# navallo/collision_avoidance

Hardware: AMD Instinct MI355X
Metric: agent-steps/sec (whole node), 4096 arenas x 64 agents per GPU (higher is better)
Workload: dtype f32

## Files before the change

collision_avoidance_amd/_lib.py:

```python
import ctypes as C
import os

from . import build as _build

OBS_DIM = 64
MAX_NEIGHBORS, MAX_OBST_NEIGHBORS, MAX_AGENTS = 16, 64, 1024
MAX_AGENTS_LARGE = 16384
CREATE_TILED = 1
CREATE_TILED_GRID = 4
CREATE_TILED_PARAMS = 16
CREATE_TILED_WIDE = 32
EDGE_GRID_MAX_EDGES, EDGE_GRID_MAX_ENTRIES = 65535, 1 << 22
DONE_XLESS, DONE_GOAL, DONE_REGOAL = 0, 1, 2
F_OBS, F_STATS, F_AUTORESET, F_NODONE, F_FREEZE = 1, 2, 4, 8, 16
F_CONTACT = 32
TRACE_POS, TRACE_VEL = 1, 2
SCN_CROWD, SCN_CIRCLE, SCN_DOORWAY, SCN_CONGESTED, SCN_INCOMING, SCN_BLOCKS, SCN_DEADLOCK, SCN_CROWD_SEPARATED = range(8)

(FLD_POS_X, FLD_POS_Y, FLD_VEL_X, FLD_VEL_Y, FLD_PREF_X, FLD_PREF_Y, FLD_GOAL_X, FLD_GOAL_Y,
 FLD_GOAL2_X, FLD_GOAL2_Y, FLD_REWARD, FLD_AGENT_DONE, FLD_ARRIVE_STEP, FLD_NB_COUNT, FLD_NB_IDX,
 FLD_OBST_COUNT, FLD_OBST_IDX, FLD_OBS, FLD_STEP_COUNT, FLD_ARENA_DONE, FLD_EPISODE,
 FLD_REGOAL_COUNT, FLD_ALAN_WEIGHTS, FLD_ALAN_TIMES, FLD_ALAN_ACTION, FLD_ARENA_STATS) = range(26)

EXPORTS = ("ca_create", "ca_destroy", "ca_last_error", "ca_set_stream", "ca_set_obstacles", "ca_init_scenario", "ca_set",
           "ca_get", "ca_field_ptr", "ca_bind_obs", "ca_reset", "ca_step", "ca_step_host", "ca_orca_step", "ca_observe", "ca_rollout",
           "ca_get_stats", "ca_reset_stats", "ca_sync", "ca_debug_math", "ca_profile", "ca_profile_read", "ca_launch_info",
           "ca_alan_configure", "ca_alan_step", "ca_alan_rollout", "ca_reset_masked", "ca_get_obstacles",
           "ca_set_obstacles_per_arena", "ca_get_obstacles_arena", "ca_solver_info", "ca_source_sha", "ca_host_alloc", "ca_host_free",
           "ca_step_packed", "ca_allow_obstacle_overflow", "ca_alan_configure_per_arena", "ca_alan_actions_arena",
           "ca_set_agent_params", "ca_get_agent_params", "ca_agent_params_info",
           "ca_set_agent_counts", "ca_get_agent_counts", "ca_agent_counts_info", "ca_create_ex", "ca_tiled_info", "ca_tiled_grid_info",
           "ca_rollout_trace", "ca_alan_rollout_trace", "ca_tiled_edge_grid", "ca_tiled_edge_grid_info", "ca_edge_grid_build",
           "ca_contacts", "ca_get_contacts", "ca_contacts_ptr",
           "ca_set_agent_sensing", "ca_get_agent_sensing", "ca_agent_sensing_info", "ca_nbr_seed_info",
           "ca_arena_gather", "ca_snapshot_create", "ca_snapshot_save", "ca_snapshot_load", "ca_snapshot_destroy",
           "ca_fork_bytes_per_arena", "ca_rollout_actions",
           "ca_policy_configure", "ca_policy_clear", "ca_policy_info", "ca_policy_actions", "ca_rollout_policy",
           "ca_nav_configure", "ca_nav_clear", "ca_nav_info", "ca_nav_get_field", "ca_nav_pref", "ca_rollout_nav", "ca_nav_mask_build")
POLICY_OUT_IDENTITY, POLICY_OUT_CLIP = 0, 1
POLICY_MAX_LAYERS, POLICY_MAX_WIDTH = 4, 128
NAV_MAX_CELLS, NAV_MAX_GOALS, NAV_MAX_LOOKAHEAD = 32768, 16, 8
NAV_STAY, NAV_NONE = 8, 9
NAV_OFFSETS = ((1, 0), (0, 1), (-1, 0), (0, -1), (1, 1), (-1, 1), (-1, -1), (1, -1))


class Config(C.Structure):
    _fields_ = [
        ("n_arenas", C.c_int32), ("n_agents", C.c_int32), ("arena_offset", C.c_int64),
        ("seed", C.c_uint64), ("reward_scale", C.c_double), ("time_step", C.c_float),
        ("neighbor_dist", C.c_float), ("max_neighbors", C.c_int32), ("time_horizon", C.c_float),
        ("time_horizon_obst", C.c_float), ("radius", C.c_float), ("max_speed", C.c_float),
        ("max_obst_neighbors", C.c_int32), ("max_step", C.c_int32), ("done_mode", C.c_int32),
        ("done_x_thresh", C.c_float), ("spawn_x0", C.c_float), ("spawn_x1", C.c_float),
        ("spawn_y0", C.c_float), ("spawn_y1", C.c_float), ("goal_x0", C.c_float),
        ("goal_x1", C.c_float), ("goal_y0", C.c_float), ("goal_y1", C.c_float),
    ]

# ... 111 lines not shown
    L.ca_nav_get_field.argtypes = [vp, i32, i32, vp, vp, vp, i32]
    L.ca_nav_pref.argtypes = [vp, vp, u32]
    L.ca_rollout_nav.argtypes = [vp, i32, u32, C.POINTER(Trace)]
    L.ca_nav_mask_build.argtypes = [vp, i32, C.c_float, C.c_float, C.c_float, i32, i32, C.c_float, vp, i32]
    L.ca_get_stats.argtypes = [vp, C.POINTER(Stats)]
    L.ca_reset_stats.argtypes = [vp]
    L.ca_sync.argtypes = [vp]
    L.ca_allow_obstacle_overflow.argtypes = [vp, i32]
    L.ca_debug_math.argtypes = [vp, i32, vp, vp, i32]
    L.ca_profile.argtypes = [vp, i32]
    L.ca_profile_read.argtypes = [vp, C.POINTER(i32), C.POINTER(C.c_float)]
    L.ca_launch_info.argtypes = [vp] + [C.POINTER(i32)] * 4
    L.ca_solver_info.argtypes = [vp, C.POINTER(i32), C.POINTER(i32)]
    L.ca_set_agent_params.argtypes = [vp, vp, vp, vp, vp, sz, i32]
    L.ca_get_agent_params.argtypes = [vp, vp, vp, vp, vp, sz, i32]
    L.ca_agent_params_info.argtypes = [vp, C.POINTER(i32)]
    L.ca_set_agent_counts.argtypes = [vp, vp, sz, i32]
    L.ca_get_agent_counts.argtypes = [vp, vp, sz, i32]
    L.ca_agent_counts_info.argtypes = [vp, C.POINTER(i32)]
    L.ca_set_agent_sensing.argtypes = [vp, vp, vp, sz, i32]
    L.ca_get_agent_sensing.argtypes = [vp, vp, vp, sz, i32]
    L.ca_agent_sensing_info.argtypes = [vp, C.POINTER(i32)]
    L.ca_nbr_seed_info.argtypes = [vp, C.POINTER(i32)]
    L.ca_arena_gather.argtypes = [vp, vp, sz, i32, u32]
    L.ca_snapshot_create.argtypes = [vp, C.POINTER(vp)]
    L.ca_snapshot_save.argtypes = [vp, vp]
    L.ca_snapshot_load.argtypes = [vp, vp, vp, sz, i32, u32]
    L.ca_snapshot_destroy.argtypes = [vp, vp]
    L.ca_fork_bytes_per_arena.argtypes = [vp, C.POINTER(sz)]
    L.ca_source_sha.argtypes = []
    L.ca_source_sha.restype = C.c_char_p
    for name in EXPORTS:
        if name not in ("ca_last_error", "ca_source_sha"):
            getattr(L, name).restype = C.c_int
    _lib = L
    return L


def edge_grid_build(edges_pq, rng):
    import numpy as np
    L = load()
    pq = np.ascontiguousarray(edges_pq, np.float32).reshape(-1, 4)
    d = EdgeGridDesc()
    ptr = pq.ctypes.data_as(C.c_void_p) if len(pq) else None
    check(L, None, L.ca_edge_grid_build(ptr, len(pq), float(rng), C.byref(d), None, 0, None, 0), "ca_edge_grid_build")
    cs, en = np.zeros(d.gx * d.gy + 1, np.uint32), np.zeros(max(1, d.n_entries), np.uint32)
# ... 20 lines not shown
```

collision_avoidance_amd/csrc/ca_common.h:

```cpp
#pragma once
#include "ca_math.h"
#include <type_traits>
#include <utility>

struct AlanArenaSets;
struct WideObstLists;
struct AgentParams;
struct ArenaCounts;
struct AgentSensing;
struct Trace;
struct ActionSeq;
struct SeededScan;

namespace ca {

template <class T, class... P> constexpr bool has_tag = (std::is_same_v<T, P> || ...);

constexpr int SMAX = 16;
constexpr int SWIDE = 64;
constexpr float EPS = 0.00001f;

struct ObstDev {
    float px, py, ux, uy;
    float qx, qy, qux, quy;
    float pux, puy;
    int next, prev;
    int convex, qconvex, pad0, pad1;
};
static_assert(sizeof(ObstDev) == 64, "edge record is one 64-byte line");

struct Line {
    V2 point, dir;
};

struct TraceDev;
// ... 259 lines not shown
```

collision_avoidance_amd/csrc/ca_env.hip:

```cpp
#include "../../include/ca_env.h"

#include <hip/hip_runtime.h>
#include <hip/hip_ext.h>

#include <algorithm>
#include <cmath>
#include <cstdarg>
#include <cstdlib>
#include <cstdio>
#include <cstring>
#include <string>
#include <vector>

#include "ca_kernels.h"
#include "ca_edge_grid_host.h"
#include "ca_nav_host.h"

using namespace ca;

struct StateSet {
    unsigned char* base = nullptr;
    unsigned char* alan = nullptr;
    int alan_nA = 0;
};
// ... 63 lines not shown
        int L = 0, P = 0, out_mode = 0, maxw = 0;
        int width[CA_POLICY_MAX_LAYERS + 1] = {0, 0, 0, 0, 0};
        float limit = 0.0f;
        unsigned wp_off[CA_POLICY_MAX_LAYERS] = {0, 0, 0, 0}, bp_off[CA_POLICY_MAX_LAYERS] = {0, 0, 0, 0}, wset = 0, bset = 0;
        float *d_wp = nullptr, *d_bp = nullptr, *act = nullptr;
        int* d_set = nullptr;
    } pol;
    struct Nav {
        bool on = false;
        float x0 = 0.0f, y0 = 0.0f, cell = 0.0f, ics = 0.0f, clearance = 0.0f;
        int gx = 0, gy = 0, G = 0, sets = 0, per_arena = 0, lookahead = 0, sweeps_max = 0, block = 0;
        float* d_dist = nullptr;
        unsigned char* d_next = nullptr;
        int* d_class = nullptr;
        std::vector<unsigned char> h_blocked;
    } nav;
    unsigned long long* ovf_host = nullptr;
    bool allow_overflow = false;
    int* d_order = nullptr;
    int P = 1, logP = 0, BS = 64, grid = 1, K = 0, S = 1;
    bool obs_dense_on = false;
    bool lists_trusted = true;
    int LS = 1, apb = 1, linv = 65536, dense = 0;
    struct { int reg_lines = -1, pair = -1, alan_fused = -1, nbr_seed = -1, nav_block = 0; } sw;
    int ST = 0, KT = 16;
    int SMX = 4;
    int max_edges = 0;
    int n_cus = 256;
    bool pair = false;
    size_t lds_p = 0;
    bool quad = false;
    bool quad_roll = false;
    int BSq = 64, grid_q = 1, SQ = 4;
    size_t lds_q = 0;
    size_t lds = 0;
    bool ap = false, quad_cfg = false, quad_roll_cfg = false;
    float* d_ap[4] = {nullptr, nullptr, nullptr, nullptr};
    float* d_ap_oct = nullptr;
    std::vector<float> h_ap[4];
    bool ac = false, ap_user = false;
    int* d_counts = nullptr;
    std::vector<int> h_counts;
    bool sens = false;
    float* d_as_nd = nullptr;
    unsigned char* d_as_k = nullptr;
    std::vector<float> h_as_nd;
    std::vector<int> h_as_k;
// ... 168 lines not shown
    c.trace = e->d_trace;
    c.actseq = e->d_actseq;
    c.as_neighbor_dist = e->sens ? e->d_as_nd : nullptr; c.as_max_neighbors = e->sens ? e->d_as_k : nullptr;
}

static void fill_args(ca_env* e, StepArgs& a, const float* actions, uint32_t flags) {
    const ca_config& c = e->cfg;
    a.pos_x = e->pos_x; a.pos_y = e->pos_y; a.vel_x = e->vel_x; a.vel_y = e->vel_y;
    a.pref_x = e->pref_x; a.pref_y = e->pref_y; a.goal_x = e->goal_x; a.goal_y = e->goal_y;
    a.counts = e->counts; a.nb_idx = e->nb_idx; a.obst_idx = e->obst_idx;
    a.arena_done = e->arena_done; a.arena_stats = e->arena_stats; a.cold = e->d_cold;
    a.obst = e->d_obst; a.tab_off = e->d_tab_off; a.actions = actions; a.alan = nullptr; a.alan_u = nullptr;
#ifdef CA_STAMPS
    a.order = e->d_order;
#endif
    a.reset_px = nullptr; a.reset_py = nullptr; a.reset_mask = nullptr; a.dbg = e->dbg;
    a.n_obst = e->h_tab_off.empty() ? (int)e->h_obst.size() : 0; a.A = c.n_arenas; a.N = c.n_agents; a.P = e->P; a.logP = e->logP;
    a.K = e->K; a.S = e->S; a.flags = flags; a.a0 = 0; a.a1 = c.n_arenas; a.T = 1;
    a.LS = e->LS; a.apb = e->apb; a.linv = e->linv; a.dense = e->dense; a.nb_hint = e->lists_trusted ? 1 : 0;
    a.time_step = c.time_step; a.neighbor_dist = c.neighbor_dist; a.time_horizon = c.time_horizon;
    a.time_horizon_obst = c.time_horizon_obst; a.radius = c.radius; a.max_speed = c.max_speed;
}

struct SolveLaunch { const void* fn; dim3 grid, block; size_t lds; bool seeded = false; };
template <class F> static const void* fn_ptr(F* f) { return reinterpret_cast<const void*>(f); }
template <int KMAX, int ST, int SMX, bool ALAN, class... PER>
static const void* step_fn_for(int BS, bool seed, bool* seeded) {
#if CA_NBR_SEED
    if (seed && BS == 64) { *seeded = true; return fn_ptr(&step_kernel<KMAX, 64, ST, SMX, ALAN, PER..., SeededScan>); }
#endif
    if constexpr (ALAN) {
        return BS == 64 ? fn_ptr(&step_kernel<KMAX, 64, ST, SMX, true, PER...>) : fn_ptr(&step_kernel<KMAX, 128, ST, SMX, true, PER...>);
    } else {
        switch (BS) {
            case 64: return fn_ptr(&step_kernel<KMAX, 64, ST, SMX>);
            case 128: return fn_ptr(&step_kernel<KMAX, 128, ST, SMX>);
            case 256: return fn_ptr(&step_kernel<KMAX, 256, ST, SMX>);
            case 512: return fn_ptr(&step_kernel<KMAX, 512, ST, SMX>);
            default: return fn_ptr(&step_kernel<KMAX, 1024, ST, SMX>);
        }
    }
}
template <int KMAX>
static const void* pair_fn_for(int BS) {
    return BS == 256 ? fn_ptr(&pair_kernel<KMAX, 256>) : fn_ptr(&pair_kernel<KMAX, 512>);
}
template <int KMAX, int SQ, bool ALAN, class... PER>
static const void* quad_fn_for(int BS) {
    switch (BS) {
        case 64: return fn_ptr(&quad_kernel<KMAX, 64, SQ, ALAN, PER...>);
        case 128: return fn_ptr(&quad_kernel<KMAX, 128, SQ, ALAN, PER...>);
        case 256: return fn_ptr(&quad_kernel<KMAX, 256, SQ, ALAN, PER...>);
// ... 22 lines not shown
    switch (BS) {
        case 64: return fn_ptr(&step_kernel<KMAX, 64, 0, SMAX, false, ArenaCounts>);
        case 128: return fn_ptr(&step_kernel<KMAX, 128, 0, SMAX, false, ArenaCounts>);
        case 256: return fn_ptr(&step_kernel<KMAX, 256, 0, SMAX, false, ArenaCounts>);
        case 512: return fn_ptr(&step_kernel<KMAX, 512, 0, SMAX, false, ArenaCounts>);
        default: return fn_ptr(&step_kernel<KMAX, 1024, 0, SMAX, false, ArenaCounts>);
    }
}
template <int KMAX, class... TAGS>
static const void* sens_fn_for(int BS) {
    switch (BS) {
        case 64: return fn_ptr(&step_kernel<KMAX, 64, 0, SMAX, false, TAGS...>);
        case 128: return fn_ptr(&step_kernel<KMAX, 128, 0, SMAX, false, TAGS...>);
        case 256: return fn_ptr(&step_kernel<KMAX, 256, 0, SMAX, false, TAGS...>);
        case 512: return fn_ptr(&step_kernel<KMAX, 512, 0, SMAX, false, TAGS...>);
        default: return fn_ptr(&step_kernel<KMAX, 1024, 0, SMAX, false, TAGS...>);
    }
}
template <class... TAGS>
static const void* sens_fn_of(const ca_env* e) {
    return e->KT == 5 ? sens_fn_for<5, TAGS...>(e->BS) : (e->KT == 16 ? sens_fn_for<16, TAGS...>(e->BS) : sens_fn_for<10, TAGS...>(e->BS));
}
template <bool ALAN, class... PER>
static const void* lane_fn_for(const ca_env* e, bool* seeded) {
    const bool sd = e->sw.nbr_seed != 0;
    if (e->sens) return e->ac ? sens_fn_of<ArenaCounts, AgentSensing>(e) : sens_fn_of<AgentSensing>(e);
    if (e->ac) return e->KT == 5 ? ac_fn_for<5>(e->BS, sd, seeded) : (e->KT == 16 ? ac_fn_for<16>(e->BS, sd, seeded) : ac_fn_for<10>(e->BS, sd, seeded));
    if (e->ap) return e->KT == 5 ? ap_fn_for<5>(e->BS) : (e->KT == 16 ? ap_fn_for<16>(e->BS) : ap_fn_for<10>(e->BS));
    if (e->SMX > SMAX) return e->KT == 5 ? wide_fn_for<5>(e->BS) : (e->KT == 16 ? wide_fn_for<16>(e->BS) : wide_fn_for<10>(e->BS));
    if (e->ST > 0 && e->SMX > 4) return e->KT == 5 ? step_fn_for<5, 4, 16, ALAN, PER...>(e->BS, sd, seeded) : step_fn_for<10, 4, 16, ALAN, PER...>(e->BS, sd, seeded);
    if (e->ST > 0) return e->KT == 5 ? step_fn_for<5, 4, 4, ALAN, PER...>(e->BS, sd, seeded) : step_fn_for<10, 4, 4, ALAN, PER...>(e->BS, sd, seeded);
    if (e->KT == 5) return step_fn_for<5, 0, SMAX, ALAN, PER...>(e->BS, sd, seeded);
    if constexpr (!ALAN) { if (e->KT == 16) return step_fn_for<16, 0, SMAX, false>(e->BS, sd, seeded); }
    return step_fn_for<10, 0, SMAX, ALAN, PER...>(e->BS, sd, seeded);
}
template <bool ALAN, class... PER>
static const void* quad_fn_for(const ca_env* e) {
    if (e->SQ > 4) return e->KT == 5 ? quad_fn_for<5, 16, ALAN, PER...>(e->BSq) : quad_fn_for<10, 16, ALAN, PER...>(e->BSq);
    return e->KT == 5 ? quad_fn_for<5, 4, ALAN, PER...>(e->BSq) : quad_fn_for<10, 4, ALAN, PER...>(e->BSq);
}
template <int KMAX, int SEARCH, class... PER>
static const void* tiled_solve_fn_for(int TILE) {
    switch (TILE) {
        case 64: return fn_ptr(&tiled_solve_kernel<KMAX, 64, SEARCH, PER...>);
        case 256: return fn_ptr(&tiled_solve_kernel<KMAX, 256, SEARCH, PER...>);
        default: return fn_ptr(&tiled_solve_kernel<KMAX, 128, SEARCH, PER...>);
    }
}
template <int SEARCH, class... PER>
static const void* tiled_solve_fn_for(const ca_env* e) {
    return e->KT == 5 ? tiled_solve_fn_for<5, SEARCH, PER...>(e->TILE)
                      : (e->KT == 16 ? tiled_solve_fn_for<16, SEARCH, PER...>(e->TILE) : tiled_solve_fn_for<10, SEARCH, PER...>(e->TILE));
}
enum { TILED_SORT_LAUNCHES = 3 };
// ... 10 lines not shown
    if (e->tgrid) return e->ap ? tiled_solve_fn_for<SEARCH_GRID, AgentParams>(e) : tiled_solve_fn_for<SEARCH_GRID>(e);
    return e->ap ? tiled_solve_fn_for<SEARCH_ALL, AgentParams>(e) : tiled_solve_fn_for<SEARCH_ALL>(e);
}
static const void* tiled_advance_fn(const ca_env* e) {
    if (e->ap) return e->egrid ? fn_ptr(&tiled_advance_kernel<true, AgentParams>) : fn_ptr(&tiled_advance_kernel<false, AgentParams>);
    return e->egrid ? fn_ptr(&tiled_advance_kernel<true>) : fn_ptr(&tiled_advance_kernel<false>);
}
static const void* tiled_close_fn(const ca_env* e) {
    if (e->sens) return fn_ptr(&tiled_close_kernel<AgentSensing>);
    return e->ap ? fn_ptr(&tiled_close_kernel<AgentParams>) : fn_ptr(&tiled_close_kernel<>);
}
static SolveLaunch solve_launch(const ca_env* e, bool alan, bool rollout, bool trace = false, bool actseq = false) {
    if (e->tiled)
        return {tiled_solve_fn(e, e->egrid), dim3(e->grid), dim3(e->TILE), e->lds};
    const bool per = alan && e->alan_per;
    if (e->quad || (rollout && e->quad_roll) || (alan && !e->alan_lane)) {
        const void* f = actseq ? quad_fn_for<false, ActionSeq>(e)
                      : trace ? (alan ? quad_fn_for<true, Trace>(e) : quad_fn_for<false, Trace>(e))
                              : (per ? quad_fn_for<true, AlanArenaSets>(e) : (alan ? quad_fn_for<true>(e) : quad_fn_for<false>(e)));
        return {f, dim3(e->grid_q), dim3(e->BSq), alan ? quad_lds_bytes(e->BSq, e->KT, e->SQ, e->n_actions) : e->lds_q};
    }
    if (e->pair)
        return {e->KT == 5 ? pair_fn_for<5>(e->BS) : pair_fn_for<10>(e->BS), dim3(e->grid), dim3(2 * e->BS), e->lds_p};
    bool seeded = false;
    const void* f = per ? lane_fn_for<true, AlanArenaSets>(e, &seeded) : (alan ? lane_fn_for<true>(e, &seeded) : lane_fn_for<false>(e, &seeded));
    return {f, dim3(e->grid), dim3(e->BS), e->lds, seeded};
}
static hipError_t allow_lds(const SolveLaunch& s) {
    return s.lds > 48 * 1024 ? hipFuncSetAttribute(s.fn, hipFuncAttributeMaxDynamicSharedMemorySize, (int)s.lds) : hipSuccess;
}
static hipError_t launch_step(ca_env* e, const StepArgs& a) {
    const SolveLaunch s = solve_launch(e, a.alan != nullptr, a.T > 1 || e->actseq_on, e->trace_on && a.T > 1, e->actseq_on);
    if (!(a.flags & CA_F_FREEZE)) e->lists_trusted = true;
    if (e->tiled) {
        TiledEdgeArgs ta;
        ta.s = a; ta.nv_x = e->nv_x; ta.nv_y = e->nv_y; ta.scr = e->tscr; ta.tiles = e->tiles;
        ta.cell_count = e->tg_count; ta.cell_start = e->tg_start; ta.key = e->tg_key;
        ta.sx = e->tg_sx; ta.sy = e->tg_sy; ta.sidx = e->tg_sidx;
        ta.gx = e->tgx; ta.gy = e->tgy; ta.ics = e->tics;
        ta.eg = e->eg.d_desc; ta.eg_cells = e->eg.d_cells; ta.eg_entries = e->eg.d_entries;
        TiledCloseParamsArgs ca;
        static_cast<TiledArgs&>(ca) = ta; ca.r_max = e->ap_rmax;
        void* params[] = {&ta};
        void* cparams[] = {&ca};
        const struct { const void* fn; dim3 grid, block; size_t lds; void** args; } seq[TILED_SORT_LAUNCHES + 3] = {
            {fn_ptr(&tiled_bin_kernel), s.grid, s.block, 0, params},
            {fn_ptr(&tiled_scan_kernel), dim3(e->cfg.n_arenas), dim3(1024), 0, params},
            {fn_ptr(&tiled_scatter_kernel), s.grid, s.block, 0, params},
            {s.fn, s.grid, s.block, s.lds, params},
// ... 319 lines not shown
                return fail(nullptr, CA_ERANGE, "ca_create: %s=%g outside the supported range [%g, %g]", q.name, (double)q.v, (double)q.lo, (double)q.hi);
        const float box[] = {cfg->spawn_x0, cfg->spawn_x1, cfg->spawn_y0, cfg->spawn_y1, cfg->goal_x0, cfg->goal_x1, cfg->goal_y0, cfg->goal_y1,
                             cfg->done_x_thresh};
        for (float v : box)
            if (!(fabsf(v) <= CA_MAX_COORD)) return fail(nullptr, CA_ERANGE, "ca_create: a spawn / goal box coordinate (%g) is beyond %g or not a number", (double)v, (double)CA_MAX_COORD);
    }
    if ((size_t)cfg->n_arenas * cfg->n_agents > (size_t)1 << 30)
        return fail(nullptr, CA_ERANGE, "ca_create: more than 2^30 agents on one handle");
    int ndev = 0;
    if (hipGetDeviceCount(&ndev) != hipSuccess || ndev <= 0)
        return fail(nullptr, CA_ENODEV, "ca_create: no HIP device (this library has no CPU path)");
    if (device < 0 || device >= ndev) return fail(nullptr, CA_ENODEV, "ca_create: device %d of %d", device, ndev);
    ca_env* e = new ca_env();
    e->cfg = *cfg;
    e->device = device;
    hipError_t r = hipSetDevice(device);
    if (r == hipSuccess) {
        if (stream) e->stream = (hipStream_t)stream;
        else { r = hipStreamCreateWithFlags(&e->stream, hipStreamNonBlocking); e->own_stream = true; }
    }
    {
        auto digit = [](const char* name) { const char* v = getenv(name); return (v && v[0] >= '0' && v[0] <= '9') ? v[0] - '0' : -1; };
        e->sw.reg_lines = digit("CA_REG_LINES"); e->sw.pair = digit("CA_PAIR"); e->sw.alan_fused = digit("CA_ALAN_FUSED");
        e->sw.nbr_seed = digit("CA_NBR_SEED");
        const char* nb = getenv("CA_NAV_BLOCK");
        e->sw.nav_block = nb ? atoi(nb) : 0;
    }
    e->tiled = tiled;
    e->twide = twide;
    if (tiled) {
        const char* v = getenv("CA_TILE");
        const int want = v ? atoi(v) : 0;
        e->TILE = (want == 64 || want == 256) ? want : 128;
        if (cfg->max_obst_neighbors > SMAX) {
            e->TILE = (want == 64 || want == 128 || want == 256) ? want : 64;
            const size_t need = tiled_lds_bytes(e->TILE, cfg->max_neighbors, cfg->max_obst_neighbors);
            if (need > LDS_PER_CU) {
                fail(nullptr, CA_ERANGE, "ca_create_ex: the tiled solve kernel for a tile of %d agents (CA_TILE), max_neighbors=%d, max_obst_neighbors=%d "
                     "does not fit the 160 KiB of LDS of a CU (%zu B: max_neighbors + max_obst_neighbors lines per lane)", e->TILE,
                     cfg->max_neighbors, cfg->max_obst_neighbors, need);
                if (e->own_stream && e->stream) hipStreamDestroy(e->stream);
                delete e;
                return CA_ERANGE;
            }
        }
        e->tiles = (cfg->n_agents + e->TILE - 1) / e->TILE;
    }
// ... 788 lines not shown
        const float* s = e->sens ? e->h_as_nd.data() : uni.data();
        if (dst_is_device) { HIPCHK(e, upload(e, neighbor_dist, s, an * 4)); }
        else memcpy(neighbor_dist, s, an * 4);
    }
    if (max_neighbors) {
        std::vector<int> uni;
        if (!e->sens) uni.assign(an, e->cfg.max_neighbors);
        const int* s = e->sens ? e->h_as_k.data() : uni.data();
        if (dst_is_device) { HIPCHK(e, upload(e, max_neighbors, s, an * 4)); }
        else memcpy(max_neighbors, s, an * 4);
    }
    return CA_OK;
}

int ca_agent_sensing_info(ca_env* e, int32_t* per_agent) {
    if (!e) return CA_EINVAL;
    if (per_agent) *per_agent = e->sens ? 1 : 0;
    return CA_OK;
}

int ca_nbr_seed_info(ca_env* e, int32_t* seeded) {
    if (!e) return CA_EINVAL;
    if (seeded) *seeded = solve_launch(e, false, false).seeded ? 1 : 0;
    return CA_OK;
}

}


static void host_scenario(const ca_env* e, int scenario, int An, std::vector<float>& px, std::vector<float>& py, std::vector<float>& vx,
                          std::vector<float>& vy, std::vector<float>& fx, std::vector<float>& fy, std::vector<double>& gx,
                          std::vector<double>& gy, std::vector<double>& g2x, std::vector<double>& g2y) {
    const ca_config& c = e->cfg;
    const int A = An, N = c.n_agents;
    const size_t an = (size_t)An * N;
    px.assign(an, 0.0f); py.assign(an, 0.0f); vx.assign(an, 0.0f); vy.assign(an, 0.0f); fx.assign(an, 0.0f); fy.assign(an, 0.0f);
    gx.assign(an, 0.0); gy.assign(an, 0.0); g2x.assign(an, 0.0); g2y.assign(an, 0.0);
    const double r = (double)c.radius;
    for (int a = 0; a < A; ++a) {
        const int64_t g = c.arena_offset + a;
        double theta = 0.0;
        for (int i = 0; i < N; ++i) {
            const size_t q = (size_t)a * N + i;
            double u0, u1, s, cs;
            rng2(c.seed, g, i, RNG_HEADING, 0, &u0, &u1);
            sincos64(uniform64(0.0, 2.0 * M_PI, u0), &s, &cs);
// ... 1869 lines not shown
```

collision_avoidance_amd/csrc/ca_lp.h:

```cpp
#pragma once
#include "ca_common.h"

namespace ca {

struct LdsLines {
    float4* base;
    int stride;
    __device__ __forceinline__ Line get(int j) const {
        const float4 v = base[j * stride];
        Line l; l.point = mk(v.x, v.y); l.dir = mk(v.z, v.w);
        return l;
    }
    __device__ __forceinline__ void put(int j, const Line& l) const {
        base[j * stride] = make_float4(l.point.x, l.point.y, l.dir.x, l.dir.y);
    }
};
struct PrivLines {
    const Line* p;
    __device__ __forceinline__ Line get(int j) const { return p[j]; }
};

template <class LS>
__device__ __forceinline__ bool lp1(const LS& ls, int lineNo, float radius, V2 opt, bool dirOpt, V2& result) {
    const Line L = ls.get(lineNo);
// ... 248 lines not shown
                        failed |= quad_xor<0xB1>(failed);
                    }
                    {
                        const float oR = quad_xor<0x4E>(tRight), oL = quad_xor<0x4E>(tLeft);
                        tRight = (oR < tRight) ? oR : tRight;
                        tLeft = (tLeft < oL) ? oL : tLeft;
                        failed |= quad_xor<0x4E>(failed);
                    }
                    if (failed || tLeft > tRight) ok = false;
                    else res = (dot(opt, L.dir) > 0.0f) ? L.point + tRight * L.dir : L.point + tLeft * L.dir;
                }
            }
            if (ok) result = res;
            distance = det(Li.dir, Li.point - result);
            wave_lds_sync();
        }
    }
    if (live && q == 0) { const lp3_v4f o = {result.x, result.y, h.z, 0.0f}; hdr[slot] = o; }
}
__device__ __forceinline__ void lp3_coop(float4* pool, int ML, int nslots, float radius, int stride = POOL_SLOTS) {
    lp3_coop_lds((lp3_lds_v4f*)pool, ML, nslots, radius, stride);
}

}
```

collision_avoidance_amd/csrc/ca_step.h:

```cpp
#pragma once
#include "ca_lp.h"
#include "ca_lines.h"
#include "ca_nbr.h"
#include "ca_rules.h"

namespace ca {

__host__ __device__ inline size_t step_lds_bytes(int BS, int K, int S, int ST = 0, int KMAX = 0) {
    if (ST > 0) return (size_t)(BS / 64) * (2 * (ST + KMAX)) * POOL_SLOTS * 16 + (size_t)BS * 32;
    return (size_t)BS * ((size_t)(K + S) * 16 + 16 + 16);
}
__host__ __device__ inline size_t step_lds_bytes_ap(int BS, int K, int S) { return step_lds_bytes(BS, K, S) + (size_t)BS * 4; }



#define CA_AS(n) __attribute__((address_space(n)))
template <bool NW16, int TS>
__device__ __noinline__ void solve_many_obstacles(CA_AS(3) char* tbl3, int MLX, const CA_AS(1) char* tab1, const CA_AS(1) char* oidx1,
                                                 const CA_AS(1) char* nidx1, int stride, int ocnt, int ncnt, const CA_AS(3) char* arena3, int bs,
                                                 V2 pos, V2 vel, V2 pref, float R, float invTO, float invT, float invDt, float max_speed) {
    float4* tbl = (float4*)tbl3;
    const ObstDev* tab = (const ObstDev*)tab1;
    const unsigned short* oidx = (const unsigned short*)oidx1;
    const void* nidx = (const void*)nidx1;
// ... 8 lines not shown
        if (obst_orca_line(tab, e, pos, vel, R, invTO, covered, line)) { ls.put(nl, line); ++nl; }
    }
    const int numObst = nl;
    for (int k = 0; k < ncnt; ++k) {
        const int j = ld_idx_t<NW16>(nidx, (size_t)k * (size_t)stride);
        ls.put(nl, agent_orca_line(pos, vel, mk(ax[j], ay[j]), mk(avx[j], avy[j]), R, invT, invDt));
        ++nl;
    }
    V2 nv = mk(0.0f, 0.0f);
    const int fail = lp2(ls, nl, max_speed, pref, false, nv);
    tbl[(2 * MLX - 1) * TS] = make_float4(nv.x, nv.y, __int_as_float(nl | (numObst << 8) | (fail << 16)), 0.0f);
}

#ifndef CA_LB512
#define CA_LB512 4
#endif
template <int KMAX, int BS, int ST, int SMX = (ST > 0 ? ST : SMAX), bool ALAN = false, class... PER>
__global__ __launch_bounds__(BS, ST > 0 ? (BS == 512 ? CA_LB512 : 4) : 1) void step_kernel(const StepArgs p) {
    constexpr int AM = !ALAN ? 0 : (has_tag<AlanArenaSets, PER...> ? 2 : 1);
    constexpr bool AC = has_tag<ArenaCounts, PER...>;
    constexpr bool AS = has_tag<AgentSensing, PER...>;
    constexpr bool AP = has_tag<AgentParams, PER...> || AC || AS;
    static_assert(!AP || (ST == 0 && !ALAN && SMX <= SMAX), "per-agent parameters: the LDS line table with lists of up to 16, no ALAN form");
    extern __shared__ float4 smem4[];
    constexpr bool LISTP = BS > 64 && !AP;
    __shared__ unsigned s_vmax2;
    if constexpr (LISTP) { if (threadIdx.x == 0) s_vmax2 = 0u; }
    CA_PRIO_START();
    nbr_body<KMAX, BS, SMX, AP, AC, AS, has_tag<SeededScan, PER...>>(p);
    constexpr int ML = ST + KMAX;
    const int tid = threadIdx.x;
    const int P = p.P;
    int la, i;
    lane_slot(p, tid, la, i);
    const int apb = p.apb;
    const int a = p.a0 + work_block(p) * apb + la;
    const bool frozen = arena_frozen(p, a);
    int n_a = p.N;
    if constexpr (AC) n_a = ((a < p.a1) && (la < apb)) ? p.cold->agent_counts[a] : 0;
    const bool active = (a < p.a1) && (i < n_a) && (la < apb) && !frozen;
    if (frozen && i == 0) p.arena_stats[(size_t)a * ST_STRIDE + ST_FROZEN] += 1;
    const int N = p.N, K = p.K, S = p.S;
    const int q = active ? a * N + i : 0;
    const int lbase = tid - i;

    float4* s_lines = smem4;
// ... 82 lines not shown
                        static_for<ST>([&](auto jc) __attribute__((always_inline)) {
                            constexpr int j = decltype(jc)::value;
                            if (j < no && line_covers(unpack_line(L[j]), c1, c2, invTO, R)) c = true;
                        });
                        return c;
                    };
                    Line line;
                    if (obst_orca_line(tab, e, pos, vel, R, invTO, covered, line)) {
                        const float4 pl = pack_line(line);
                        static_for<ST>([&](auto jc) __attribute__((always_inline)) {
                            constexpr int j = decltype(jc)::value;
                            if (j == no) L[j] = pl;
                        });
                        ++no;
                    }
                }
            }
        }
#if defined(CA_STAMPS) && CA_STAMPS == 3
        if ((tid & 63) == 0 && p.dbg) p.dbg[((size_t)blockIdx.x * (BS / 64) + (tid >> 6)) * 16 + 4] = 0;
#else
        CA_STAMP(4);
#endif
        CA_PRIO_POINT(2);
        {
            const float invT = 1.0f / p.time_horizon;
            const float invDt = 1.0f / p.time_step;
            int jn[KMAX];
            static_for<KMAX>([&](auto kc) __attribute__((always_inline)) {
                constexpr int k = decltype(kc)::value;
                jn[k] = (k < ncnt) ? ld_idx_t<CA_NBW16(BS)>(nb_idx_s, ((size_t)a * K + k) * N + i) : 0;
            });
            static_for<KMAX>([&](auto kc) __attribute__((always_inline)) {
                constexpr int k = decltype(kc)::value;
                if (k < ncnt) {
                    const int j = lbase + jn[k];
                    L[ST + k] = pack_line(agent_orca_line(pos, vel, mk(s_px[j], s_py[j]), mk(s_vx[j], s_vy[j]), R, invT, invDt));
                }
            });
        }
        CA_STAMP(5);
        CA_PRIO_POINT(3);
        const int nl = no + ncnt;
        int fail = nl;
        auto opt_fn = [&]() __attribute__((always_inline)) -> V2 {
            if constexpr (PARK_PREF) return mk(reinterpret_cast<const float*>(s_misc)[tid * 4 + 2], reinterpret_cast<const float*>(s_misc)[tid * 4 + 3]);
            else return pref;
        };
        if (fast) fail = lp2_reg<ML, ST>(L, no, ncnt, p.max_speed, opt_fn, nv);
        CA_STAMP(6);
        CA_PRIO_POINT(5);
        {
            float4* pool = s_lines + (size_t)(tid >> 6) * (2 * ML) * POOL_SLOTS;
            float4* hdr = pool + (size_t)(2 * ML - 1) * POOL_SLOTS;
            bool need = active && fail < nl;
            const unsigned long long below = (1ull << (tid & 63)) - 1ull;
            while (true) {
                const unsigned long long m = __ballot(need);
#if defined(CA_STAMPS) && CA_STAMPS == 3
                if ((tid & 63) == 0 && p.dbg) p.dbg[((size_t)blockIdx.x * (BS / 64) + (tid >> 6)) * 16 + 4] += 1 + ((unsigned long long)__popcll(m) << 32);
#endif
                if (__builtin_expect(!m, 1)) break;
                const int rank = __popcll(m & below);
                const bool mine = need && rank < POOL_SLOTS;
                if (mine) {
                    LdsLines pls; pls.base = pool + rank; pls.stride = POOL_SLOTS;
                    static_for<ML>([&](auto kc) __attribute__((always_inline)) {
                        constexpr int k = decltype(kc)::value;
                        const bool valid = (k < ST) ? (k < no) : (k - ST < ncnt);
                        if (valid) pls.base[((k < ST) ? k : no + (k - ST)) * POOL_SLOTS] = L[k];
                    });
                    hdr[rank] = make_float4(nv.x, nv.y, __int_as_float(nl | (no << 8) | (fail << 16)), 0.0f);
                }
                wave_lds_sync();
                const int waiting = __popcll(m);
                lp3_coop(pool, ML, waiting < POOL_SLOTS ? waiting : POOL_SLOTS, p.max_speed);
                wave_lds_sync();
                if (mine) {
                    const float4 h = hdr[rank];
                    nv = mk(h.x, h.y);
                    need = false;
                }
            }
            if constexpr (SMX > ST) {
                constexpr int MLX = SMX + KMAX;
                constexpr int GX = (2 * ML * POOL_SLOTS) / (2 * MLX);
                static_assert(GX >= 1 && GX <= POOL_SLOTS, "the many-obstacle tables fit the wave's pool");
                int tid_o = threadIdx.x;
                asm volatile("" : "+v"(tid_o));
                int la_o, i_o;
                lane_slot(p, tid_o, la_o, i_o);
                const int a_o = p.a0 + work_block(p) * apb + la_o;
                const bool act_o = (a_o < p.a1) && (i_o < N) && (la_o < apb) && !arena_frozen(p, a_o);
                const int cnts_o = act_o ? (int)p.counts[a_o * N + i_o] : 0;
                bool need_o = (cnts_o >> 8) > ST;
                const unsigned long long below_o = (1ull << (tid_o & 63)) - 1ull;
                float rad_o = p.radius, tho_o = p.time_horizon_obst, th_o = p.time_horizon, dt_o = p.time_step, ms_o = p.max_speed;
                asm volatile("" : "+s"(rad_o), "+s"(tho_o), "+s"(th_o), "+s"(dt_o), "+s"(ms_o));
                while (true) {
                    const unsigned long long om = __ballot(need_o);
                    if (__builtin_expect(!om, 1)) break;
                    const int rank = __popcll(om & below_o);
                    const bool mine = need_o && rank < GX;
                    if (mine) {
// ... 305 lines not shown
```

collision_avoidance_amd/vec_env.py:

```python
import ctypes as C

import numpy as np

from . import _lib, scenarios

try:
    import torch
except Exception:
    torch = None

_I32_FIELDS = {_lib.FLD_AGENT_DONE, _lib.FLD_ARRIVE_STEP, _lib.FLD_NB_COUNT, _lib.FLD_NB_IDX,
               _lib.FLD_OBST_COUNT, _lib.FLD_OBST_IDX, _lib.FLD_STEP_COUNT, _lib.FLD_ARENA_DONE,
               _lib.FLD_EPISODE, _lib.FLD_REGOAL_COUNT, _lib.FLD_ALAN_ACTION}
_ARENA_FIELDS = {_lib.FLD_STEP_COUNT, _lib.FLD_ARENA_DONE, _lib.FLD_EPISODE}
DEFAULT_MAX_OBST_NEIGHBORS = 16
_F64_FIELDS = {_lib.FLD_GOAL_X, _lib.FLD_GOAL_Y, _lib.FLD_GOAL2_X, _lib.FLD_GOAL2_Y, _lib.FLD_ALAN_WEIGHTS,
               _lib.FLD_ALAN_TIMES}


def _ptr(a):
    return a.ctypes.data_as(C.c_void_p)


_TRACE_CHANNELS = {"pos": _lib.TRACE_POS, "vel": _lib.TRACE_VEL}
# ... 467 lines not shown
        n = (C.c_int32 * 4)()
        ms = (C.c_float * 4)()
        self._call("ca_profile_read", self.h, n, ms)
        return {k: (n[i], ms[i]) for i, k in enumerate(("nbr_kernel", "step_kernel", "obs_kernel", "reset_kernels"))}

    def launch_info(self):
        v = [C.c_int32() for _ in range(4)]
        self._call("ca_launch_info", self.h, *[C.byref(x) for x in v])
        lanes, roll = C.c_int32(), C.c_int32()
        self._call("ca_solver_info", self.h, C.byref(lanes), C.byref(roll))
        per, cnt, sen = C.c_int32(), C.c_int32(), C.c_int32()
        self._call("ca_agent_params_info", self.h, C.byref(per))
        self._call("ca_agent_counts_info", self.h, C.byref(cnt))
        self._call("ca_agent_sensing_info", self.h, C.byref(sen))
        return dict(block=v[0].value, grid=v[1].value, lds_bytes=v[2].value, obs_grid=v[3].value,
                    lanes_per_agent=lanes.value, rollout_one_launch=roll.value, agent_params=bool(per.value),
                    agent_counts=bool(cnt.value), agent_sensing=bool(sen.value))

    def nbr_seed_info(self):
        v = C.c_int32()
        self._call("ca_nbr_seed_info", self.h, C.byref(v))
        return bool(v.value)

    def tiled_info(self):
        v = [C.c_int32() for _ in range(4)]
        self._call("ca_tiled_info", self.h, *[C.byref(x) for x in v])
        return dict(tiled=bool(v[0].value), tile_agents=v[1].value, tiles_per_arena=v[2].value, launches_per_step=v[3].value)

    def tiled_grid_info(self):
        v = [C.c_int32() for _ in range(3)] + [C.c_float(), C.c_int32()]
        self._call("ca_tiled_grid_info", self.h, *[C.byref(x) for x in v])
        return dict(grid=bool(v[0].value), cells_x=v[1].value, cells_y=v[2].value, cell_size=v[3].value, sort_launches=v[4].value)

    def set_edge_grid(self, on=True):
        self._call("ca_tiled_edge_grid", self.h, 1 if on else 0)

    def edge_grid_info(self, arena=0):
        v = [C.c_int32() for _ in range(3)] + [C.c_float(), C.c_float(), C.c_int32()]
        self._call("ca_tiled_edge_grid_info", self.h, int(arena), *[C.byref(x) for x in v])
        return dict(on=v[0].value, cells_x=v[1].value, cells_y=v[2].value, cell_size_x=v[3].value, cell_size_y=v[4].value,
                    entries=v[5].value)

    _AGENT_PARAMS = ("radius", "max_speed", "time_horizon", "time_horizon_obst")

    def set_agent_params(self, radius=None, max_speed=None, time_horizon=None, time_horizon_obst=None):
        keep, ptrs = [], []
# ... 547 lines not shown
```

include/ca_env.h:

```cpp
#ifndef CA_ENV_H
#define CA_ENV_H

#include <stddef.h>
#include <stdint.h>

#ifdef __cplusplus
extern "C" {
#endif

#define CA_OBS_DIM 64
#define CA_N_RAYS 16
#define CA_MAX_NEIGHBORS 16
#define CA_MAX_OBST_NEIGHBORS 64
#define CA_MAX_AGENTS 1024
#define CA_MAX_AGENTS_LARGE 16384

#define CA_CREATE_TILED 1u
#define CA_CREATE_TILED_GRID 4u
#define CA_CREATE_TILED_PARAMS 16u
#define CA_CREATE_TILED_WIDE 32u

#define CA_OK 0
#define CA_EINVAL (-1)
#define CA_ENODEV (-2)
// ... 91 lines not shown
int ca_set_stream(ca_env* env, void* stream);

int ca_set_obstacles(ca_env* env, const float* verts_xy, const int32_t* poly_sizes, int32_t n_poly);
int ca_get_obstacles(ca_env* env, float* verts_xy, int32_t* next, int32_t* convex, int32_t cap, int32_t* n_out);
int ca_set_obstacles_per_arena(ca_env* env, const float* verts_xy, const int32_t* poly_sizes, const int32_t* n_poly);
int ca_get_obstacles_arena(ca_env* env, int32_t arena, float* verts_xy, int32_t* next, int32_t* convex, int32_t cap,
                           int32_t* n_out);

int ca_set_agent_params(ca_env* env, const float* radius, const float* max_speed, const float* time_horizon,
                        const float* time_horizon_obst, size_t bytes_each, int32_t src_is_device);
int ca_get_agent_params(ca_env* env, float* radius, float* max_speed, float* time_horizon,
                        float* time_horizon_obst, size_t bytes_each, int32_t dst_is_device);
int ca_agent_params_info(ca_env* env, int32_t* per_agent);

int ca_set_agent_counts(ca_env* env, const int32_t* counts, size_t bytes, int32_t src_is_device);
int ca_get_agent_counts(ca_env* env, int32_t* counts, size_t bytes, int32_t dst_is_device);
int ca_agent_counts_info(ca_env* env, int32_t* per_arena);

int ca_set_agent_sensing(ca_env* env, const float* neighbor_dist, const int32_t* max_neighbors, size_t bytes_each, int32_t src_is_device);
int ca_get_agent_sensing(ca_env* env, float* neighbor_dist, int32_t* max_neighbors, size_t bytes_each, int32_t dst_is_device);
int ca_agent_sensing_info(ca_env* env, int32_t* per_agent);

int ca_nbr_seed_info(ca_env* env, int32_t* seeded);

int ca_init_scenario(ca_env* env, int32_t scenario);

int ca_set(ca_env* env, int32_t field, const void* src, size_t bytes, int32_t src_is_device);
int ca_get(ca_env* env, int32_t field, void* dst, size_t bytes, int32_t dst_is_device);
int ca_host_alloc(ca_env* env, size_t bytes, void** out);
int ca_host_free(ca_env* env, void* p);
int ca_field_ptr(ca_env* env, int32_t field, void** dev_ptr, size_t* bytes);
int ca_bind_obs(ca_env* env, void* dev_ptr, size_t bytes);

int ca_reset(ca_env* env, const float* pos_x, const float* pos_y, int32_t pos_is_device, uint32_t flags);

int ca_reset_masked(ca_env* env, const int32_t* mask, int32_t mask_is_device, uint32_t flags);

int ca_step(ca_env* env, const float* actions, uint32_t flags);
int ca_step_host(ca_env* env, const float* actions_host, uint32_t flags);
int ca_step_packed(ca_env* env, const float* actions_host, uint32_t flags, void* out_host, size_t out_bytes);
int ca_orca_step(ca_env* env, uint32_t flags);
int ca_observe(ca_env* env);
int ca_contacts(ca_env* env);
int ca_get_contacts(ca_env* env, int32_t* agents, int32_t* wall, int32_t* nearest, float* nearest_d2, float* wall_d2, size_t bytes_each,
                    int32_t dst_is_device);
int ca_contacts_ptr(ca_env* env, void** dev_ptr, size_t* bytes);
// ... 149 lines not shown
```

Baseline: 2.584 billion.

## Add paired-lane LP3 fallback solving up to 32 agents with two lanes each

Adds a new LP3 (3D linear program fallback) variant in which two lanes cooperate on one agent, splitting the projected-line construction and the inner intersection loop and combining the results with DPP and quad swizzles. When more agents need LP3 than the single-lane pool holds but no more than 32, the iterative pool loop stops early and one paired round solves them all at once. This is meant to remove extra serialized pool rounds inside the wave. In exchange it adds register pressure, more cross-lane traffic, and a new kernel instantiation; it is enabled by default only for the register-line, seeded, non-ALAN BS=64 path.

```diff
diff --git a/collision_avoidance_amd/_lib.py b/collision_avoidance_amd/_lib.py
--- a/collision_avoidance_amd/_lib.py
+++ b/collision_avoidance_amd/_lib.py
@@ -32,7 +32,7 @@
            "ca_set_agent_counts", "ca_get_agent_counts", "ca_agent_counts_info", "ca_create_ex", "ca_tiled_info", "ca_tiled_grid_info",
            "ca_rollout_trace", "ca_alan_rollout_trace", "ca_tiled_edge_grid", "ca_tiled_edge_grid_info", "ca_edge_grid_build",
            "ca_contacts", "ca_get_contacts", "ca_contacts_ptr",
-           "ca_set_agent_sensing", "ca_get_agent_sensing", "ca_agent_sensing_info", "ca_nbr_seed_info",
+           "ca_set_agent_sensing", "ca_get_agent_sensing", "ca_agent_sensing_info", "ca_nbr_seed_info", "ca_lp3_pairs_info",
            "ca_arena_gather", "ca_snapshot_create", "ca_snapshot_save", "ca_snapshot_load", "ca_snapshot_destroy",
            "ca_fork_bytes_per_arena", "ca_rollout_actions",
            "ca_policy_configure", "ca_policy_clear", "ca_policy_info", "ca_policy_actions", "ca_rollout_policy",
@@ -190,6 +190,7 @@
     L.ca_get_agent_sensing.argtypes = [vp, vp, vp, sz, i32]
     L.ca_agent_sensing_info.argtypes = [vp, C.POINTER(i32)]
     L.ca_nbr_seed_info.argtypes = [vp, C.POINTER(i32)]
+    L.ca_lp3_pairs_info.argtypes = [vp, C.POINTER(i32)]
     L.ca_arena_gather.argtypes = [vp, vp, sz, i32, u32]
     L.ca_snapshot_create.argtypes = [vp, C.POINTER(vp)]
     L.ca_snapshot_save.argtypes = [vp, vp]
diff --git a/collision_avoidance_amd/csrc/ca_common.h b/collision_avoidance_amd/csrc/ca_common.h
--- a/collision_avoidance_amd/csrc/ca_common.h
+++ b/collision_avoidance_amd/csrc/ca_common.h
@@ -11,6 +11,7 @@
 struct Trace;
 struct ActionSeq;
 struct SeededScan;
+struct PairedLp3;
 
 namespace ca {
 
diff --git a/collision_avoidance_amd/csrc/ca_env.hip b/collision_avoidance_amd/csrc/ca_env.hip
--- a/collision_avoidance_amd/csrc/ca_env.hip
+++ b/collision_avoidance_amd/csrc/ca_env.hip
@@ -109,7 +109,7 @@
     bool obs_dense_on = false;
     bool lists_trusted = true;
     int LS = 1, apb = 1, linv = 65536, dense = 0;
-    struct { int reg_lines = -1, pair = -1, alan_fused = -1, nbr_seed = -1, nav_block = 0; } sw;
+    struct { int reg_lines = -1, pair = -1, alan_fused = -1, nbr_seed = -1, lp3_pairs = -1, nav_block = 0; } sw;
     int ST = 0, KT = 16;
     int SMX = 4;
     int max_edges = 0;
@@ -324,12 +324,20 @@
     a.time_horizon_obst = c.time_horizon_obst; a.radius = c.radius; a.max_speed = c.max_speed;
 }
 
-struct SolveLaunch { const void* fn; dim3 grid, block; size_t lds; bool seeded = false; };
+struct SolveLaunch { const void* fn; dim3 grid, block; size_t lds; bool seeded = false, paired = false; };
 template <class F> static const void* fn_ptr(F* f) { return reinterpret_cast<const void*>(f); }
 template <int KMAX, int ST, int SMX, bool ALAN, class... PER>
-static const void* step_fn_for(int BS, bool seed, bool* seeded) {
+static const void* step_fn_for(int BS, bool seed, bool* seeded, bool pairs = false, bool* paired = nullptr) {
 #if CA_NBR_SEED
-    if (seed && BS == 64) { *seeded = true; return fn_ptr(&step_kernel<KMAX, 64, ST, SMX, ALAN, PER..., SeededScan>); }
+    if (seed && BS == 64) {
+        *seeded = true;
+#if CA_LP3_PAIRS
+        if constexpr (ST > 0 && SMX == ST && !ALAN && sizeof...(PER) == 0) {
+            if (pairs && paired) { *paired = true; return fn_ptr(&step_kernel<KMAX, 64, ST, SMX, false, SeededScan, PairedLp3>); }
+        }
+#endif
+        return fn_ptr(&step_kernel<KMAX, 64, ST, SMX, ALAN, PER..., SeededScan>);
+    }
 #endif
     if constexpr (ALAN) {
         return BS == 64 ? fn_ptr(&step_kernel<KMAX, 64, ST, SMX, true, PER...>) : fn_ptr(&step_kernel<KMAX, 128, ST, SMX, true, PER...>);
@@ -398,14 +406,15 @@
     return e->KT == 5 ? sens_fn_for<5, TAGS...>(e->BS) : (e->KT == 16 ? sens_fn_for<16, TAGS...>(e->BS) : sens_fn_for<10, TAGS...>(e->BS));
 }
 template <bool ALAN, class... PER>
-static const void* lane_fn_for(const ca_env* e, bool* seeded) {
+static const void* lane_fn_for(const ca_env* e, bool* seeded, bool* paired) {
     const bool sd = e->sw.nbr_seed != 0;
+    const bool pl = e->sw.lp3_pairs < 0 ? CA_LP3_PAIRS_DEFAULT != 0 : e->sw.lp3_pairs != 0;
     if (e->sens) return e->ac ? sens_fn_of<ArenaCounts, AgentSensing>(e) : sens_fn_of<AgentSensing>(e);
     if (e->ac) return e->KT == 5 ? ac_fn_for<5>(e->BS, sd, seeded) : (e->KT == 16 ? ac_fn_for<16>(e->BS, sd, seeded) : ac_fn_for<10>(e->BS, sd, seeded));
     if (e->ap) return e->KT == 5 ? ap_fn_for<5>(e->BS) : (e->KT == 16 ? ap_fn_for<16>(e->BS) : ap_fn_for<10>(e->BS));
     if (e->SMX > SMAX) return e->KT == 5 ? wide_fn_for<5>(e->BS) : (e->KT == 16 ? wide_fn_for<16>(e->BS) : wide_fn_for<10>(e->BS));
     if (e->ST > 0 && e->SMX > 4) return e->KT == 5 ? step_fn_for<5, 4, 16, ALAN, PER...>(e->BS, sd, seeded) : step_fn_for<10, 4, 16, ALAN, PER...>(e->BS, sd, seeded);
-    if (e->ST > 0) return e->KT == 5 ? step_fn_for<5, 4, 4, ALAN, PER...>(e->BS, sd, seeded) : step_fn_for<10, 4, 4, ALAN, PER...>(e->BS, sd, seeded);
+    if (e->ST > 0) return e->KT == 5 ? step_fn_for<5, 4, 4, ALAN, PER...>(e->BS, sd, seeded, pl, paired) : step_fn_for<10, 4, 4, ALAN, PER...>(e->BS, sd, seeded, pl, paired);
     if (e->KT == 5) return step_fn_for<5, 0, SMAX, ALAN, PER...>(e->BS, sd, seeded);
     if constexpr (!ALAN) { if (e->KT == 16) return step_fn_for<16, 0, SMAX, false>(e->BS, sd, seeded); }
     return step_fn_for<10, 0, SMAX, ALAN, PER...>(e->BS, sd, seeded);
@@ -462,9 +471,9 @@
     }
     if (e->pair)
         return {e->KT == 5 ? pair_fn_for<5>(e->BS) : pair_fn_for<10>(e->BS), dim3(e->grid), dim3(2 * e->BS), e->lds_p};
-    bool seeded = false;
-    const void* f = per ? lane_fn_for<true, AlanArenaSets>(e, &seeded) : (alan ? lane_fn_for<true>(e, &seeded) : lane_fn_for<false>(e, &seeded));
-    return {f, dim3(e->grid), dim3(e->BS), e->lds, seeded};
+    bool seeded = false, paired = false;
+    const void* f = per ? lane_fn_for<true, AlanArenaSets>(e, &seeded, &paired) : (alan ? lane_fn_for<true>(e, &seeded, &paired) : lane_fn_for<false>(e, &seeded, &paired));
+    return {f, dim3(e->grid), dim3(e->BS), e->lds, seeded, paired};
 }
 static hipError_t allow_lds(const SolveLaunch& s) {
     return s.lds > 48 * 1024 ? hipFuncSetAttribute(s.fn, hipFuncAttributeMaxDynamicSharedMemorySize, (int)s.lds) : hipSuccess;
@@ -830,7 +839,7 @@
     {
         auto digit = [](const char* name) { const char* v = getenv(name); return (v && v[0] >= '0' && v[0] <= '9') ? v[0] - '0' : -1; };
         e->sw.reg_lines = digit("CA_REG_LINES"); e->sw.pair = digit("CA_PAIR"); e->sw.alan_fused = digit("CA_ALAN_FUSED");
-        e->sw.nbr_seed = digit("CA_NBR_SEED");
+        e->sw.nbr_seed = digit("CA_NBR_SEED"); e->sw.lp3_pairs = digit("CA_LP3_PAIRS");
         const char* nb = getenv("CA_NAV_BLOCK");
         e->sw.nav_block = nb ? atoi(nb) : 0;
     }
@@ -1665,6 +1674,12 @@
 int ca_nbr_seed_info(ca_env* e, int32_t* seeded) {
     if (!e) return CA_EINVAL;
     if (seeded) *seeded = solve_launch(e, false, false).seeded ? 1 : 0;
+    return CA_OK;
+}
+
+int ca_lp3_pairs_info(ca_env* e, int32_t* paired) {
+    if (!e) return CA_EINVAL;
+    if (paired) *paired = solve_launch(e, false, false).paired ? 1 : 0;
     return CA_OK;
 }
 
diff --git a/collision_avoidance_amd/csrc/ca_lp.h b/collision_avoidance_amd/csrc/ca_lp.h
--- a/collision_avoidance_amd/csrc/ca_lp.h
+++ b/collision_avoidance_amd/csrc/ca_lp.h
@@ -294,4 +294,106 @@
     lp3_coop_lds((lp3_lds_v4f*)pool, ML, nslots, radius, stride);
 }
 
-}
+#ifndef CA_LP3_PAIRS
+#define CA_LP3_PAIRS 1
+#endif
+#ifndef CA_LP3_PAIRS_DEFAULT
+#define CA_LP3_PAIRS_DEFAULT 1
+#endif
+constexpr int PAIR_SLOTS = 32;
+template <bool ODD>
+__device__ __forceinline__ float lp3_pair_bcast(float v) {
+    return __int_as_float(__builtin_amdgcn_update_dpp(0, __float_as_int(v), ODD ? 0xF5 : 0xA0, 0xF, 0xF, false));
+}
+template <int ML>
+__device__ __forceinline__ void lp3_pair_lds(lp3_lds_v4f* pool, lp3_lds_v4f* hdr, int nslots, float radius) {
+    constexpr int NP = ML - 1;
+    constexpr int NR = (NP + 1) / 2;
+    const int lane = threadIdx.x & 63, slot = lane >> 1, hh = lane & 1;
+    Lds3Lines ls; ls.base = pool + slot; ls.stride = PAIR_SLOTS;
+    const bool live = slot < nslots;
+    lp3_v4f h = {0.0f, 0.0f, 0.0f, 0.0f};
+    if (live) h = hdr[slot];
+    const int packed = __float_as_int(h.z);
+    const int n = live ? (packed & 0xFF) : 0, numObst = (packed >> 8) & 0xFF, begin = (packed >> 16) & 0xFF;
+    V2 result = mk(h.x, h.y);
+    float distance = 0.0f;
+    for (int i = begin; i < n; ++i) {
+        const Line Li = ls.get(i);
+        if (det(Li.dir, Li.point - result) > distance) {
+            lp3_v4f P[NR];
+            unsigned own = 0u;
+            static_for<NR>([&](auto sc) __attribute__((always_inline)) {
+                constexpr int s = decltype(sc)::value;
+                const int p = 2 * s + hh;
+                lp3_v4f v = {0.0f, 0.0f, 1.0f, 0.0f};
+                bool valid = p < numObst || p < i;
+                if (valid) {
+                    const Line Lj = ls.get(p);
+                    Line l = Lj;
+                    if (p >= numObst) {
+                        const float d = det(Li.dir, Lj.dir);
+                        if (fabsf(d) <= EPS) {
+                            if (dot(Li.dir, Lj.dir) > 0.0f) valid = false;
+                            else l.point = 0.5f * (Li.point + Lj.point);
+                        } else {
+                            l.point = Li.point + div_ir(det(Lj.dir, Li.point - Lj.point), d) * Li.dir;
+                        }
+                        l.dir = normalize_ir(Lj.dir - Li.dir);
+                    }
+                    if (valid) { v.x = l.point.x; v.y = l.point.y; v.z = l.dir.x; v.w = l.dir.y; }
+                }
+                P[s] = v;
+                own |= valid ? (1u << p) : 0u;
+            });
+            const unsigned have = own | (unsigned)quad_xor<0xB1>((int)own);
+            const V2 opt = mk(-Li.dir.y, Li.dir.x);
+            V2 res = opt * radius;
+            bool ok = true;
+            static_for<NP>([&](auto ic) __attribute__((always_inline)) {
+                constexpr int ii = decltype(ic)::value;
+                if (ok && ((have >> ii) & 1u)) {
+                    Line L;
+                    L.point = mk(lp3_pair_bcast<(ii & 1) != 0>(P[ii >> 1].x), lp3_pair_bcast<(ii & 1) != 0>(P[ii >> 1].y));
+                    L.dir = mk(lp3_pair_bcast<(ii & 1) != 0>(P[ii >> 1].z), lp3_pair_bcast<(ii & 1) != 0>(P[ii >> 1].w));
+                    if (det(L.dir, L.point - res) > 0.0f) {
+                        const float dp = dot(L.point, L.dir);
+                        const float disc = sqr(dp) + sqr(radius) - absSq(L.point);
+                        int failed = disc < 0.0f ? 1 : 0;
+                        const float sq = sqrt_ir(disc);
+                        float tLeft = -dp - sq;
+                        float tRight = -dp + sq;
+                        static_for<(ii + 1) / 2>([&](auto jc) __attribute__((always_inline)) {
+                            constexpr int sj = decltype(jc)::value;
+                            const int jj = 2 * sj + hh;
+                            const bool on = (jj < ii) & (((own >> jj) & 1u) != 0u);
+                            const Line M = unpack_line(make_float4(P[sj].x, P[sj].y, P[sj].z, P[sj].w));
+                            const float den = det(L.dir, M.dir);
+                            const float num = det(M.dir, L.point - M.point);
+                            const bool par = fabsf(den) <= EPS;
+                            const float t = div_ir(num, den);
+                            const bool pos = den >= 0.0f;
+                            const bool right = on & !par & pos, left = on & !par & !pos;
+                            tRight = (right & (t < tRight)) ? t : tRight;
+                            tLeft = (left & (tLeft < t)) ? t : tLeft;
+                            failed |= (on & par & (num < 0.0f)) ? 1 : 0;
+                        });
+                        {
+                            const float oR = quad_xor<0xB1>(tRight), oL = quad_xor<0xB1>(tLeft);
+                            tRight = (oR < tRight) ? oR : tRight;
+                            tLeft = (tLeft < oL) ? oL : tLeft;
+                            failed |= quad_xor<0xB1>(failed);
+                        }
+                        if (failed || tLeft > tRight) ok = false;
+                        else res = (dot(opt, L.dir) > 0.0f) ? L.point + tRight * L.dir : L.point + tLeft * L.dir;
+                    }
+                }
+            });
+            if (ok) result = res;
+            distance = det(Li.dir, Li.point - result);
+        }
+    }
+    if (live && hh == 0) { const lp3_v4f o = {result.x, result.y, h.z, 0.0f}; hdr[slot] = o; }
+}
+
+}
diff --git a/collision_avoidance_amd/csrc/ca_step.h b/collision_avoidance_amd/csrc/ca_step.h
--- a/collision_avoidance_amd/csrc/ca_step.h
+++ b/collision_avoidance_amd/csrc/ca_step.h
@@ -54,6 +54,9 @@
     constexpr bool AS = has_tag<AgentSensing, PER...>;
     constexpr bool AP = has_tag<AgentParams, PER...> || AC || AS;
     static_assert(!AP || (ST == 0 && !ALAN && SMX <= SMAX), "per-agent parameters: the LDS line table with lists of up to 16, no ALAN form");
+    constexpr bool PL = has_tag<PairedLp3, PER...>;
+    static_assert(!PL || (CA_LP3_PAIRS && BS == 64 && ST > 0 && SMX == ST && !ALAN && !AP),
+                  "the paired LP3 round: one wave, register lines, no many-obstacle stage (it reads the staged velocities the headers overwrite), no ALAN form");
     extern __shared__ float4 smem4[];
     constexpr bool LISTP = BS > 64 && !AP;
     __shared__ unsigned s_vmax2;
@@ -182,6 +185,12 @@
 #else
         CA_STAMP(4);
 #endif
+#if defined(CA_STAMPS) && CA_STAMPS < 3
+        unsigned long long* const lp3_cnt = p.dbg ? p.dbg + ((size_t)((p.A + p.apb - 1) / p.apb + blockIdx.x) * (BS / 64) + (tid >> 6)) * 16 + 2 : nullptr;
+        if ((tid & 63) == 0 && lp3_cnt) *lp3_cnt = 0;
+#elif defined(CA_STAMPS) && CA_STAMPS == 3
+        unsigned long long* const lp3_cnt = p.dbg ? p.dbg + ((size_t)blockIdx.x * (BS / 64) + (tid >> 6)) * 16 + 4 : nullptr;
+#endif
         CA_PRIO_POINT(2);
         {
             const float invT = 1.0f / p.time_horizon;
@@ -217,10 +226,13 @@
             const unsigned long long below = (1ull << (tid & 63)) - 1ull;
             while (true) {
                 const unsigned long long m = __ballot(need);
-#if defined(CA_STAMPS) && CA_STAMPS == 3
-                if ((tid & 63) == 0 && p.dbg) p.dbg[((size_t)blockIdx.x * (BS / 64) + (tid >> 6)) * 16 + 4] += 1 + ((unsigned long long)__popcll(m) << 32);
+#if defined(CA_STAMPS) && CA_STAMPS <= 3
+                if ((tid & 63) == 0 && lp3_cnt) *lp3_cnt += 1 + ((unsigned long long)__popcll(m) << 32);
 #endif
                 if (__builtin_expect(!m, 1)) break;
+                if constexpr (PL) {
+                    if (__popcll(m) > POOL_SLOTS && __popcll(m) <= PAIR_SLOTS) break;
+                }
                 const int rank = __popcll(m & below);
                 const bool mine = need && rank < POOL_SLOTS;
                 if (mine) {
@@ -240,6 +252,31 @@
                     const float4 h = hdr[rank];
                     nv = mk(h.x, h.y);
                     need = false;
+                }
+            }
+            if constexpr (PL) {
+                const unsigned long long m = __ballot(need);
+                if (m != 0ull) {
+#if defined(CA_STAMPS) && CA_STAMPS <= 3
+                    if ((tid & 63) == 0 && lp3_cnt) *lp3_cnt += 1ull << 16;
+#endif
+                    float4* hdr2 = reinterpret_cast<float4*>(s_vx);
+                    const int rank = __popcll(m & below);
+                    if (need) {
+                        static_for<ML>([&](auto kc) __attribute__((always_inline)) {
+                            constexpr int k = decltype(kc)::value;
+                            const bool valid = (k < ST) ? (k < no) : (k - ST < ncnt);
+                            if (valid) pool[((k < ST) ? k : no + (k - ST)) * PAIR_SLOTS + rank] = L[k];
+                        });
+                        hdr2[rank] = make_float4(nv.x, nv.y, __int_as_float(nl | (no << 8) | (fail << 16)), 0.0f);
+                    }
+                    wave_lds_sync();
+                    lp3_pair_lds<ML>((lp3_lds_v4f*)pool, (lp3_lds_v4f*)hdr2, __popcll(m), p.max_speed);
+                    wave_lds_sync();
+                    if (need) {
+                        const float4 h = hdr2[rank];
+                        nv = mk(h.x, h.y);
+                    }
                 }
             }
             if constexpr (SMX > ST) {
diff --git a/collision_avoidance_amd/vec_env.py b/collision_avoidance_amd/vec_env.py
--- a/collision_avoidance_amd/vec_env.py
+++ b/collision_avoidance_amd/vec_env.py
@@ -513,6 +513,11 @@
         self._call("ca_nbr_seed_info", self.h, C.byref(v))
         return bool(v.value)
 
+    def lp3_pairs_info(self):
+        v = C.c_int32()
+        self._call("ca_lp3_pairs_info", self.h, C.byref(v))
+        return bool(v.value)
+
     def tiled_info(self):
         v = [C.c_int32() for _ in range(4)]
         self._call("ca_tiled_info", self.h, *[C.byref(x) for x in v])
diff --git a/include/ca_env.h b/include/ca_env.h
--- a/include/ca_env.h
+++ b/include/ca_env.h
@@ -137,6 +137,8 @@
 int ca_agent_sensing_info(ca_env* env, int32_t* per_agent);
 
 int ca_nbr_seed_info(ca_env* env, int32_t* seeded);
+
+int ca_lp3_pairs_info(ca_env* env, int32_t* paired);
 
 int ca_init_scenario(ca_env* env, int32_t scenario);
 
```

After: 2.646 billion (median of 6 runs). 1.02x the previous value.
